# PJLab-ADG/nr3d_lib

Hardware: AMD Instinct MI355X
Metric: Mpoints/s LoTD fwd+bwd (16-lvl hash) + Mrays/s march+composite, 1 & 8 GPU (higher is better)
Workload: dtype f32; 1 GPU; configs[1]: 16-level Hash LoTD (gen_ngp_cfg: T=2^19, F=2, 6 Dense + 10 Hash), 2^20 points/GPU, fwd(+dy/dx) + dL/dx + dL/dparam, fp32; points_per_gpu=1048576, n_params=12131648, parallelism=single GPU

## Files before the change

### include/nr3d_hip.h

```cpp
#ifndef NR3D_HIP_H
#define NR3D_HIP_H
#include <stdint.h>

#ifdef __cplusplus
extern "C" {
#endif

enum { NR3D_F32 = 0, NR3D_F16 = 1, NR3D_F64 = 2, NR3D_I32 = 3, NR3D_I64 = 4, NR3D_U8 = 5, NR3D_I16 = 6, NR3D_I8 = 7 };

#define NR3D_ABI_VERSION 24

const char *nr3d_last_error(void);
int nr3d_abi_version(void);

enum {
	NR3D_PROF_LOTD_FWD = 0,
	NR3D_PROF_LOTD_FWD_LDS = 1,
	NR3D_PROF_LOTD_CONTRACT_DX = 2,
	NR3D_PROF_LOTD_BIN = 3,
	NR3D_PROF_LOTD_ACCUM = 4,
	NR3D_PROF_MARCH = 5,
	NR3D_PROF_COMPOSITE_FWD = 6,
	NR3D_PROF_COMPOSITE_BWD = 7,
	NR3D_PROF_LOTD_DIRECT = 8,
	NR3D_PROF_COUNT = 9
// ... 11 lines not shown
	NR3D_OPT_FWD_SPLIT = 6,
	NR3D_OPT_FWD_LDS_STAGE = 7,
	NR3D_OPT_HVP_LEVELS = 8,
	NR3D_OPT_HVP_PAIRLANE = 9,
	NR3D_OPT_HVP_SPLIT = 10,
	NR3D_OPT_VM_SPLIT = 11,
	NR3D_OPT_CP_DIRECT = 12,
	NR3D_OPT_MARCH_GROUP = 13,
	NR3D_OPT_PACK_SCAN = 14,
	NR3D_OPT_SORT_WAVE = 15,
	NR3D_OPT_VM_DIRECT = 16,
	NR3D_OPT_DIRECT_FIXED = 17,
	NR3D_OPT_VM_SORTED = 18,
	NR3D_OPT_MLP_X3 = 19,
	NR3D_OPT_PAIR_FOLD = 20,
	NR3D_OPT_COUNT = 21
};
int nr3d_set_option(int id, int64_t value);
int64_t nr3d_get_option(int id);

#define NR3D_LOTD_MAX_LEVELS 32
#define NR3D_LOTD_MAX_DIMS 4
#define NR3D_LOTD_MAX_PSEUDO 256

enum {
	NR3D_LOD_Dense = 0, NR3D_LOD_VectorMatrix = 1, NR3D_LOD_VecZMatXoY = 2, NR3D_LOD_CP = 3,
	NR3D_LOD_CPfast = 4, NR3D_LOD_NPlaneMul = 5, NR3D_LOD_NPlaneSum = 6, NR3D_LOD_Hash = 7
};

typedef struct nr3d_lotd_level {
	uint32_t res[NR3D_LOTD_MAX_DIMS];
// ... 37 lines not shown
                     void *dL_dy_T ,
                     int32_t max_level, void *fold ,
                     void *stream);

uint64_t nr3d_lotd_dparam_workspace_bytes(const nr3d_lotd_meta_t *meta, uint32_t n_points, uint32_t n_batches);
void nr3d_lotd_set_dparam_chunk_log2(int log2_points);

int nr3d_lotd_dLdy_feature_major(uint32_t n_points, uint32_t n_encoded_dims, int grad_dtype, const void *dL_dy,
                                 int64_t g_sn, int64_t g_se, float *out, void *stream);

int nr3d_lotd_half_params_ok(const nr3d_lotd_meta_t *meta, int batched);
int nr3d_lotd_pair_path_ok(const nr3d_lotd_meta_t *meta);
int nr3d_lotd_pair_direct_levels(const nr3d_lotd_meta_t *meta, uint32_t n_points);
uint64_t nr3d_lotd_fwd_lds_levels(const nr3d_lotd_meta_t *meta, uint32_t n_points);
uint64_t nr3d_lotd_pair_fold_bytes(const nr3d_lotd_meta_t *meta, uint32_t n_points, int32_t max_level);

int nr3d_lotd_bwd_dparam(const nr3d_lotd_meta_t *meta, const void *meta_dev, uint32_t n_points,
                         int grad_dtype, const void *dL_dy, int64_t dldy_sn, int64_t dldy_se,
                         const void *dL_ddLdx, const void *x, int param_dtype, const void *params,
                         const int64_t *batch_inds, const int64_t *batch_offsets, uint32_t batch_data_size, uint32_t n_batches,
                         int32_t min_level, int32_t max_level, int out_dtype, int assign, void *dL_dparam,
                         void *workspace, uint64_t workspace_bytes, void *fold, void *stream);

int nr3d_lotd_bwd_bwd_ddLdy(const nr3d_lotd_meta_t *meta, uint32_t n_points, int x_dtype, int param_dtype,
                            const void *dL_ddLdx, const void *dy_dx, int64_t dydx_sn, int64_t dydx_se,
                            void *dL_ddLdy, int64_t out_sn, int64_t out_se, void *stream);
uint64_t nr3d_lotd_bwd_bwd_dx_workspace_bytes(const nr3d_lotd_meta_t *meta, uint32_t n_points);
int nr3d_lotd_bwd_bwd_dx(const nr3d_lotd_meta_t *meta, const void *meta_dev, uint32_t n_points,
                         int x_dtype, int param_dtype, const void *dL_ddLdx,
                         const void *dL_dy, int64_t dldy_sn, int64_t dldy_se, const void *x,
// ... 377 lines not shown
```

### nr3d_lib_amd/_abi.py

```python
ABI_VERSION = 24
SIGNATURES = {
    'nr3d_abi_version': ('int', []),
    'nr3d_alpha_to_vw_backward': ('int', ['uint32_t', 'uint64_t', 'ptr', 'ptr', 'ptr', 'ptr', 'float', 'float', 'ptr', 'ptr']),
    'nr3d_alpha_to_vw_forward': ('int', ['uint32_t', 'uint64_t', 'ptr', 'ptr', 'float', 'float', 'ptr', 'ptr', 'ptr', 'ptr']),
    'nr3d_arange_num_steps': ('int', ['uint32_t', 'int', 'ptr', 'ptr', 'ptr', 'double', 'ptr', 'ptr']),
    'nr3d_forest_identify': ('int', ['ptr', 'uint64_t', 'ptr', 'ptr', 'ptr']),
    'nr3d_forest_ray_marching_count': ('int', ['ptr', 'uint32_t', 'ptr', 'ptr', 'ptr', 'ptr', 'ptr', 'ptr', 'ptr', 'ptr', 'ptr', 'ptr', 'float', 'float', 'float', 'uint32_t', 'ptr', 'ptr', 'ptr', 'ptr']),
    'nr3d_forest_ray_marching_emit': ('int', ['ptr', 'uint32_t', 'ptr', 'ptr', 'ptr', 'ptr', 'ptr', 'ptr', 'ptr', 'ptr', 'ptr', 'ptr', 'float', 'float', 'float', 'ptr', 'ptr', 'ptr', 'ptr', 'ptr', 'ptr', 'ptr']),
    'nr3d_freq_encode_bwd': ('int', ['uint64_t', 'uint32_t', 'uint32_t', 'uint32_t', 'ptr', 'ptr', 'int64_t', 'ptr', 'ptr']),
    'nr3d_freq_encode_bwd_bwd': ('int', ['uint64_t', 'uint32_t', 'uint32_t', 'uint32_t', 'ptr', 'ptr', 'ptr', 'int64_t', 'ptr', 'ptr', 'ptr']),
    'nr3d_freq_encode_fwd': ('int', ['uint64_t', 'uint32_t', 'uint32_t', 'uint32_t', 'ptr', 'ptr', 'int64_t', 'ptr']),
    'nr3d_get_option': ('int64_t', ['int']),
    'nr3d_interleave_linstep': ('int', ['uint32_t', 'int', 'ptr', 'ptr', 'ptr', 'double', 'double', 'ptr', 'ptr', 'ptr']),
    'nr3d_last_error': ('str', []),
    'nr3d_lotd_bwd_bwd_ddLdy': ('int', ['ptr', 'uint32_t', 'int', 'int', 'ptr', 'ptr', 'int64_t', 'int64_t', 'ptr', 'int64_t', 'int64_t', 'ptr']),
    'nr3d_lotd_bwd_bwd_dx': ('int', ['ptr', 'ptr', 'uint32_t', 'int', 'int', 'ptr', 'ptr', 'int64_t', 'int64_t', 'ptr', 'ptr', 'ptr', 'ptr', 'uint32_t', 'int32_t', 'ptr', 'ptr', 'uint64_t', 'ptr']),
    'nr3d_lotd_bwd_bwd_dx_workspace_bytes': ('uint64_t', ['ptr', 'uint32_t']),
    'nr3d_lotd_bwd_dparam': ('int', ['ptr', 'ptr', 'uint32_t', 'int', 'ptr', 'int64_t', 'int64_t', 'ptr', 'ptr', 'int', 'ptr', 'ptr', 'ptr', 'uint32_t', 'uint32_t', 'int32_t', 'int32_t', 'int', 'int', 'ptr', 'ptr', 'uint64_t', 'ptr', 'ptr']),
    'nr3d_lotd_bwd_dx': ('int', ['ptr', 'uint32_t', 'int', 'int', 'ptr', 'int64_t', 'int64_t', 'ptr', 'int64_t', 'int64_t', 'ptr', 'ptr', 'int32_t', 'ptr', 'ptr']),
    'nr3d_lotd_dLdy_feature_major': ('int', ['uint32_t', 'uint32_t', 'int', 'ptr', 'int64_t', 'int64_t', 'ptr', 'ptr']),
    'nr3d_lotd_dparam_workspace_bytes': ('uint64_t', ['ptr', 'uint32_t', 'uint32_t']),
    'nr3d_lotd_forest_bwd_bwd_dx': ('int', ['ptr', 'ptr', 'ptr', 'uint32_t', 'ptr', 'ptr', 'ptr', 'ptr', 'int', 'ptr', 'ptr', 'uint32_t', 'int32_t', 'ptr', 'ptr']),
    'nr3d_lotd_forest_bwd_dparam': ('int', ['ptr', 'ptr', 'ptr', 'uint32_t', 'ptr', 'ptr', 'ptr', 'ptr', 'int', 'ptr', 'ptr', 'uint32_t', 'int32_t', 'ptr', 'ptr', 'uint64_t', 'ptr']),
    'nr3d_lotd_forest_dparam_workspace_bytes': ('uint64_t', ['ptr', 'uint32_t', 'uint32_t']),
    'nr3d_lotd_forest_fwd': ('int', ['ptr', 'ptr', 'ptr', 'uint32_t', 'ptr', 'ptr', 'int', 'ptr', 'ptr', 'uint32_t', 'int32_t', 'ptr', 'int64_t', 'int64_t', 'ptr', 'int64_t', 'int64_t', 'ptr']),
    'nr3d_lotd_fwd': ('int', ['ptr', 'ptr', 'uint32_t', 'int', 'int', 'ptr', 'ptr', 'ptr', 'ptr', 'uint32_t', 'int32_t', 'ptr', 'int64_t', 'int64_t', 'ptr', 'int64_t', 'int64_t', 'ptr']),
    'nr3d_lotd_fwd_lds_levels': ('uint64_t', ['ptr', 'uint32_t']),
    'nr3d_lotd_grid_index': ('int', ['ptr', 'ptr', 'uint32_t', 'int', 'ptr', 'ptr', 'ptr', 'uint32_t', 'int32_t', 'ptr', 'ptr']),
    'nr3d_lotd_half_params_ok': ('int', ['ptr', 'int']),
    'nr3d_lotd_meta_create': ('int', ['int32_t', 'uint32_t', 'ptr', 'ptr', 'ptr', 'uint32_t', 'int', 'ptr']),
    'nr3d_lotd_meta_regroup': ('int', ['ptr', 'uint32_t', 'uint32_t', 'ptr']),
    'nr3d_lotd_pair_direct_levels': ('int', ['ptr', 'uint32_t']),
    'nr3d_lotd_pair_fold_bytes': ('uint64_t', ['ptr', 'uint32_t', 'int32_t']),
    'nr3d_lotd_pair_path_ok': ('int', ['ptr']),
    'nr3d_lotd_set_dparam_chunk_log2': ('void', ['int']),
    'nr3d_march_composite_bwd': ('int', ['uint32_t', 'ptr', 'ptr', 'ptr', 'ptr', 'ptr', 'float', 'float', 'int', 'ptr', 'ptr', 'ptr', 'ptr', 'ptr', 'ptr', 'ptr', 'ptr', 'ptr', 'ptr', 'uint64_t', 'ptr', 'ptr']),
    'nr3d_march_composite_fwd': ('int', ['uint32_t', 'ptr', 'ptr', 'ptr', 'ptr', 'ptr', 'ptr', 'ptr', 'int', 'float', 'float', 'float', 'uint32_t', 'ptr', 'ptr', 'ptr', 'ptr', 'ptr', 'ptr', 'uint64_t', 'uint64_t', 'ptr', 'ptr', 'ptr', 'ptr', 'ptr', 'ptr', 'ptr', 'ptr', 'uint64_t', 'ptr', 'float', 'float', 'int', 'ptr', 'ptr', 'ptr', 'ptr', 'ptr', 'ptr']),
    'nr3d_march_finish_samples': ('int', ['uint64_t', 'ptr', 'ptr', 'ptr', 'ptr', 'ptr', 'ptr', 'ptr', 'ptr', 'ptr']),
    'nr3d_mark_pack_boundaries': ('int', ['uint64_t', 'int', 'ptr', 'ptr', 'ptr']),
    'nr3d_merge_pack_union': ('int', ['uint32_t', 'ptr', 'ptr', 'uint32_t', 'ptr', 'ptr', 'ptr', 'ptr', 'ptr', 'ptr', 'ptr', 'ptr', 'ptr', 'ptr', 'ptr', 'ptr']),
    'nr3d_mlp_backward': ('int', ['ptr', 'uint64_t', 'ptr', 'int64_t', 'int64_t', 'ptr', 'int64_t', 'ptr', 'ptr', 'int64_t', 'int64_t', 'ptr', 'ptr', 'ptr']),
    'nr3d_mlp_backward_backward': ('int', ['ptr', 'uint64_t', 'ptr', 'int64_t', 'int64_t', 'ptr', 'int64_t', 'ptr', 'int64_t', 'int64_t', 'ptr', 'ptr', 'int64_t', 'ptr', 'ptr']),
    'nr3d_mlp_backward_backward_ok': ('int', ['ptr']),
    'nr3d_mlp_backward_packed_floats': ('uint64_t', ['ptr']),
    'nr3d_mlp_forward': ('int', ['ptr', 'uint64_t', 'ptr', 'int64_t', 'int64_t', 'ptr', 'ptr', 'int64_t', 'ptr']),
    'nr3d_mlp_half_backward': ('int', ['ptr', 'uint64_t', 'ptr', 'int64_t', 'int64_t', 'ptr', 'int64_t', 'ptr', 'ptr', 'int64_t', 'int64_t', 'ptr', 'ptr', 'ptr']),
    'nr3d_mlp_half_backward_packed_bytes': ('uint64_t', ['ptr']),
    'nr3d_mlp_half_forward': ('int', ['ptr', 'uint64_t', 'ptr', 'int64_t', 'int64_t', 'ptr', 'ptr', 'int64_t', 'ptr']),
# ... 75 lines not shown
```

### nr3d_lib_amd/_hip.py

```python
import ctypes as C
import os
import subprocess
import threading

import torch

from nr3d_lib_amd import _abi

_PKG = os.path.dirname(os.path.abspath(__file__))
LIB_PATH = os.path.join(_PKG, "libnr3d_hip.so")
ABI_VERSION = _abi.ABI_VERSION
CSRC = os.path.join(_PKG, "csrc")

F32, F16, F64, I32, I64, U8, I16, I8 = range(8)
DTYPE_CODE = {
    torch.float32: F32, torch.float16: F16, torch.float64: F64, torch.int32: I32, torch.int64: I64,
    torch.uint8: U8, torch.bool: U8, torch.int16: I16, torch.int8: I8,
}

_lib = None
_lock = threading.Lock()


def build(verbose=False, jobs=None):
# ... 91 lines not shown
def prof_enable(*names):
    mask = 0
    for n in names:
        mask |= 1 << PROF_IDS[n]
    lib().nr3d_prof_enable(mask)


def prof_read(name, reset=True):
    ms, n = C.c_double(0.0), C.c_uint32(0)
    check(lib().nr3d_prof_read(PROF_IDS[name], C.byref(ms), C.byref(n), 1 if reset else 0))
    return float(ms.value), int(n.value)


OPTION_IDS = dict(lotd_pair=0, pair_quad=1, pair_second=2, pair_direct=3, pair_fixed=4, fwd_pairlane=5, fwd_split=6,
                  fwd_lds_stage=7, hvp_levels=8, hvp_pairlane=9, hvp_split=10, vm_split=11, cp_direct=12, march_group=13,
                  pack_scan=14, sort_wave=15, vm_direct=16, direct_fixed=17, vm_sorted=18, mlp_x3=19, pair_fold=20)


def set_option(name, value):
    l = lib()
    check(l.nr3d_set_option(OPTION_IDS[name], -1 if value is None else int(value)))


def get_option(name):
    l = lib()
    return int(l.nr3d_get_option(OPTION_IDS[name]))


class options:

    def __init__(self, **kw):
# ... 193 lines not shown
```

### nr3d_lib_amd/bindings/_lotd.py

```python
import ctypes as C
import enum

import torch

from .. import _hip as H

MAX_LEVELS, MAX_DIMS, MAX_PSEUDO = 32, 4, 256


class LoDType(enum.IntEnum):
    Dense = 0
    VectorMatrix = 1
    VecZMatXoY = 2
    CP = 3
    CPfast = 4
    NPlaneMul = 5
    NPlaneSum = 6
    Hash = 7


class InterpolationType(enum.IntEnum):
    Linear = 0
    Smoothstep = 1

# ... 340 lines not shown
            if need_param_grad and level_buckets is not None and on_bucket is not None:
                for k, (lo, hi) in enumerate(level_buckets):
                    on_bucket(k, dL_dparam[m.level_offsets[int(lo)]:m.level_offsets[min(int(hi), m.n_levels - 1) + 1]])
            return (_cast(dL_dx, input.dtype), _cast(dL_dparam, params.dtype))
        g32 = dL_dy.detach() if native else _f32c(dL_dy.detach())
        gcode = H.F16 if native else H.F32
        gsn, gse = _strides2(g32)
        st = H.stream_of(input)
        tag = ("dx" if need_input_grad else "") + ("dp" if need_param_grad else "")
        with _Prof(m, f"LoTD{D}-bwd-{tag}", N):
            gT = fold = None
            if need_input_grad and N > 0:
                j, jsn, jse = _jac_view(dy_dx.detach(), N, E, D)
                if (need_param_grad and not batched and USE_BINNED_DPARAM and gse == 1 and gsn == E
                        and g32.data_ptr() % 16 == 0):
                    gT = H.empty((E, N), dtype=torch.float32, device=dev)
                    if typed:
                        nfold = H.lib().nr3d_lotd_pair_fold_bytes(C.byref(m._cmeta()), N, max_level)
                        if nfold:
                            fold = H.empty(((nfold + 3) // 4,), dtype=torch.int32, device=dev)
                H.check(H.lib().nr3d_lotd_bwd_dx(
                    C.byref(m._cmeta()), N, H.F32, gcode, H.ptr(g32), gsn, gse, H.ptr(j), jsn, jse, H.ptr(dL_dx), H.ptr(gT),
                    max_level, H.ptr(fold), st))
            if need_param_grad and N > 0:
                x32, (p32, pcode) = _f32c(input.detach()), _ptab(params)
                nbat = _n_batches(m, p32, batch_offsets, batched)
                ws, wsb = _dparam_workspace(m, N, dev, nbat)
                if gT is not None:
                    g32, gsn, gse, gcode = gT, 1, N, H.F32
                ranges = [(0, max_level)]
                if level_buckets is not None:
                    if batched:
                        raise RuntimeError("bwd: level_buckets need non-batched params")
                    if params.dtype != torch.float32:
                        raise RuntimeError("bwd: level_buckets need float params (the slices handed out are the result)")
# ... 119 lines not shown
```

### nr3d_lib_amd/csrc/host_api.hip

```cpp
#include "common.h"
#include <string.h>
#include <limits>
#include <chrono>
#include <mutex>
#include <vector>

namespace nr3d {

static thread_local char g_err[512] = {0};

char *err_buf() { return g_err; }

int fail(const char *fmt, ...) {
	va_list ap;
	va_start(ap, fmt);
	vsnprintf(g_err, sizeof(g_err), fmt, ap);
	va_end(ap);
	return 1;
}

namespace prof {
uint32_t g_mask = 0;
struct Pair { hipEvent_t a, b; };
static std::mutex g_mu;
// ... 12 lines not shown
	g_open[id] = p; g_is_open[id] = true;
}
void end(int id, hipStream_t st) {
	std::lock_guard<std::mutex> lk(g_mu);
	if (id < 0 || id >= NR3D_PROF_COUNT || !g_is_open[id]) return;
	g_is_open[id] = false;
	if (hipEventRecord(g_open[id].b, st) == hipSuccess) g_done[id].push_back(g_open[id]);
}
}

namespace opt {
static const int64_t kDefault[NR3D_OPT_COUNT] = {
	 1,  1,  1,  1,  1,  1,
	 1,  1,  1,  1,  1,  1,
	 1,  0,  1,  1,  1,  1,
	 1,  1,  1,
};
std::atomic<int64_t> g_val[NR3D_OPT_COUNT];
static const bool g_val_init = [] {
	for (int i = 0; i < NR3D_OPT_COUNT; ++i) g_val[i].store(kDefault[i], std::memory_order_relaxed);
	return true;
}();
}

}

using namespace nr3d;

extern "C" void nr3d_prof_enable(uint32_t mask) { prof::g_mask = mask; }

extern "C" int nr3d_prof_read(int id, double *total_ms, uint32_t *n_intervals, int reset) {
// ... 167 lines not shown
```

### nr3d_lib_amd/csrc/lotd.hip

```cpp
#include "lotd_device.h"
#include <stdlib.h>
#include <vector>
#include <type_traits>
#include <algorithm>

namespace nr3d {
namespace lotd {

template <typename YT> __device__ __forceinline__ void store_nt(YT *p, float v);

template <int D, int G, bool DYDX, bool DH, int ONLY = -1, typename PT = float>
__global__ __launch_bounds__(kBlock) void k_fwd(Sched s, const nr3d_lotd_meta_t *__restrict__ md, uint32_t N,
                                                int32_t max_level, uint32_t smooth, const float *__restrict__ x,
                                                const PT *__restrict__ params, Batch ba, uint32_t vec_ok,
                                                PT *__restrict__ y, int64_t y_sn, int64_t y_se,
                                                float *__restrict__ dydx, int64_t d_sn, int64_t d_se) {
	uint32_t q, chunk;
	if (!decode_block(s, blockIdx.x, q, chunk)) return;
	const uint32_t i = chunk * kBlock + threadIdx.x;
	if (i >= N) return;
	const uint32_t level = meta_level_of(md, q);
	const uint32_t foff0 = meta_cnt_of(md, q) * G;
	const uint32_t out0 = meta_col_of(md, q);

// ... 993 lines not shown
	for (uint32_t e = 0; e < E; ++e) {
		const float g = gy[(int64_t)e * g_se];
		const float *j = jj + (int64_t)e * d_se;
#pragma unroll
		for (int d = 0; d < D; ++d) acc[d] = __fmaf_rn(g, j[d], acc[d]);
	}
#pragma unroll
	for (int d = 0; d < D; ++d) dL_dx[(size_t)i * D + d] = acc[d];
}

template <int D, typename GT>
__global__ __launch_bounds__(kBlock) void k_contract_dx_rowmajor(uint32_t N, uint32_t E, const GT *__restrict__ dL_dy,
                                                                 const float *__restrict__ dydx, int64_t d_sn,
                                                                 int64_t d_se, float *__restrict__ dL_dx,
                                                                 float *__restrict__ dL_dy_T, uint32_t *__restrict__ fold,
                                                                 uint32_t gcols, uint32_t n_zero, uint32_t slot_off) {
	constexpr int TE = 32;
	__shared__ float tile[TE][kBlock + 1];
	__shared__ uint32_t gred[kBlock / 64];
	const uint32_t i0 = blockIdx.x * kBlock, i = i0 + threadIdx.x;
	const uint32_t n_here = min((uint32_t)kBlock, N - i0);
	uint32_t gbits = 0;
	auto gm = [&](uint32_t e, float v) { if (e < gcols) gbits = max(gbits, __float_as_uint(v) & 0x7FFFFFFFu); };
	if (fold && blockIdx.x == 0)
		for (uint32_t k = threadIdx.x; k < n_zero; k += kBlock) fold[k] = 0u;
	float acc[D];
#pragma unroll
	for (int d = 0; d < D; ++d) acc[d] = 0.0f;
	for (uint32_t e0 = 0; e0 < E; e0 += TE) {
		const uint32_t te = min((uint32_t)TE, E - e0);
		if (te == TE && (E & 3u) == 0u) {
// ... 14 lines not shown
				}
			}
		} else {
			for (uint32_t v = threadIdx.x; v < kBlock * te; v += kBlock) {
				const uint32_t p = v / te, e = v - p * te;
				if (p < n_here) {
					tile[e][p] = to_f32<GT>(dL_dy[(size_t)(i0 + p) * E + e0 + e]);
					if (fold) gm(e0 + e, tile[e][p]);
				}
			}
		}
		__syncthreads();
		if (dL_dy_T && i < N) {
#pragma unroll 8
			for (uint32_t e = 0; e < te; ++e) __builtin_nontemporal_store(tile[e][threadIdx.x], &dL_dy_T[(size_t)(e0 + e) * N + i]);
		}
		if (i < N) {
			const float *jj = dydx + (int64_t)i * d_sn + (int64_t)e0 * d_se;
#pragma unroll 8
			for (uint32_t e = 0; e < te; ++e) {
				const float g = tile[e][threadIdx.x];
				const float *j = jj + (int64_t)e * d_se;
#pragma unroll
				for (int d = 0; d < D; ++d) acc[d] = __fmaf_rn(g, __builtin_nontemporal_load(j + d), acc[d]);
			}
		}
		__syncthreads();
	}
	if (i < N) {
#pragma unroll
// ... 381 lines not shown
}

extern "C" int nr3d_lotd_bwd_dx(const nr3d_lotd_meta_t *meta, uint32_t N, int x_dtype, int param_dtype, const void *dL_dy,
                                int64_t g_sn, int64_t g_se, const void *dy_dx, int64_t d_sn, int64_t d_se, void *dL_dx,
                                void *dL_dy_T, int32_t max_level, void *fold_buf, void *stream) {
	NR3D_CHECK(meta != nullptr, "LoTD: meta is NULL");
	NR3D_CHECK(x_dtype == NR3D_F32 && (param_dtype == NR3D_F32 || param_dtype == NR3D_F16), "LoTD::bwd_dx: f32 x, f32 / f16 dL_dy");
	if (N == 0) return 0;
	NR3D_CHECK(dL_dy && dy_dx && dL_dx, "LoTDEncoding::bwd: need `dy_dx` to comput `dL_dx`.");
	const uint32_t E = meta->n_encoded_dims;
	const bool g_half = param_dtype == NR3D_F16;
	const bool row_major = (g_se == 1 && g_sn == (int64_t)E && ((uintptr_t)dL_dy % (g_half ? 8 : 16)) == 0);
	NR3D_CHECK(dL_dy_T == nullptr || row_major, "LoTD::bwd_dx: dL_dy_T needs a contiguous, 16-byte aligned [N, E] dL_dy");
	NR3D_CHECK(!g_half || (row_major && (E & 3u) == 0u), "LoTD::bwd_dx: half dL_dy must be a contiguous [N, E] tensor, E % 4 == 0");
	uint32_t gcols = 0, n_zero = 0, slot_off = 0;
	uint32_t *fold = (fold_buf && pair_fold_layout(meta, N, max_level, gcols, n_zero, slot_off) != 0) ? (uint32_t *)fold_buf : nullptr;
	NR3D_CHECK(!fold || row_major, "LoTD::bwd_dx: the hand-over buffer needs a contiguous, 16-byte aligned [N, E] dL_dy");
	prof::Scope ps(NR3D_PROF_LOTD_CONTRACT_DX, (hipStream_t)stream);
	DISPATCH_D(meta->n_dims_to_encode, {
		if (row_major && g_half)
			hipLaunchKernelGGL((k_contract_dx_rowmajor<D, __half>), dim3(div_up(N, kBlock)), dim3(kBlock), 0, (hipStream_t)stream, N, E,
			                   (const __half *)dL_dy, (const float *)dy_dx, d_sn, d_se, (float *)dL_dx, (float *)dL_dy_T, fold, gcols,
			                   n_zero, slot_off);
		else if (row_major)
			hipLaunchKernelGGL((k_contract_dx_rowmajor<D, float>), dim3(div_up(N, kBlock)), dim3(kBlock), 0, (hipStream_t)stream, N, E,
			                   (const float *)dL_dy, (const float *)dy_dx, d_sn, d_se, (float *)dL_dx, (float *)dL_dy_T, fold, gcols,
			                   n_zero, slot_off);
		else
			hipLaunchKernelGGL(k_contract_dx<D>, dim3(div_up(N, kBlock)), dim3(kBlock), 0, (hipStream_t)stream, N, E,
			                   (const float *)dL_dy, g_sn, g_se, (const float *)dy_dx, d_sn, d_se, (float *)dL_dx);
	});
	NR3D_LAUNCH_CHECK();
	return 0;
}

extern "C" uint64_t nr3d_lotd_pair_fold_bytes(const nr3d_lotd_meta_t *meta, uint32_t N, int32_t max_level) {
	uint32_t gcols, n_zero, slot_off;
	return meta ? pair_fold_layout(meta, N, max_level, gcols, n_zero, slot_off) : 0;
}

extern "C" int nr3d_lotd_bwd_dparam(const nr3d_lotd_meta_t *meta, const void *meta_dev, uint32_t N, int grad_dtype,
                                    const void *dL_dy, int64_t g_sn, int64_t g_se, const void *dL_ddLdx, const void *x,
// ... 216 lines not shown
```

### nr3d_lib_amd/csrc/lotd_bin.hip

```cpp
#include "lotd_vm.h"
#include "lotd_sorted.h"
#include <stdlib.h>
#include <type_traits>

#ifndef NR3D_BIN_LDS_KB
#define NR3D_BIN_LDS_KB 72
#define NR3D_BIN_MAX_BP 512
#endif
namespace nr3d {
namespace lotd {

constexpr int kAccThreads = 1024;
constexpr int kLdsDoubles = 16384;
constexpr int kRedSlots = 4;
#ifndef NR3D_BALLOT_RANK_BUCKETS
#define NR3D_BALLOT_RANK_BUCKETS 4
#endif
constexpr uint32_t kBallotRankBuckets = NR3D_BALLOT_RANK_BUCKETS;
constexpr int kMaxPlanLevels = 64;
constexpr uint32_t kMaxBuckets = 8192;
constexpr int kBinLdsDyn = NR3D_BIN_LDS_KB * 1024 + (int)(kMaxBuckets + 1) * 4;

#define DISPATCH_DG_BIN(D_, G_, ...)                                                 \
	do {                                                                             \
// ... 1519 lines not shown
		                    : p.dL_dy + (int64_t)p0 * p.g_sn;
		c.gc = c.g_rows;
		c.sn = p.g_sn; c.se = p.g_se;
		c.ba = p.batch;
		if (c.ba.inds) c.ba.inds += p0;
		c.ba.first_point = p0;
		bool gt_ready = !row_major;
		auto need_gt = [&]() {
			if (gt_ready) return;
			if (p.g_half) launch_transpose<__half>(n, E, reinterpret_cast<const __half *>(c.g_rows), p.g_sn, p.g_se, c.gt, p.st);
			else launch_transpose<float>(n, E, c.g_rows, p.g_sn, p.g_se, c.gt, p.st);
			c.gc = c.gt; c.sn = 1; c.se = (int64_t)n;
			gt_ready = true;
		};
		if (use_pair) {
			need_gt();
			NR3D_TRY(pair_chunk(p, c));
			continue;
		}
		uint64_t served = 0;
		if (plain) {
			CpPlan cp;
			uint32_t max_acc = 0;
			if ((served = cp_plan(meta, n, p.min_level, p.max_level, lay.part_bytes / 4, cp, max_acc))) {
				need_gt();
				NR3D_TRY(cp_direct_route(p, c, cp, max_acc));
			}
		}
		if (!p.g_half) {
			VsPlan vsp;
			const uint64_t smask = vm_sorted_plan(meta, n, p.n_batches, forest, p.min_level, p.max_level, served, vsp);
// ... 33 lines not shown
```

### nr3d_lib_amd/csrc/lotd_device.h

```cpp
#pragma once
#include "common.h"
#include <type_traits>

namespace nr3d {
namespace lotd {

constexpr int kBlock = 256;
constexpr uint32_t kPrimes[7] = {1u, 2654435761u, 805459861u, 3674653429u, 2097192037u, 1434869437u, 2165219737u};

constexpr int kSchedSegs = 16;
struct Sched {
	uint32_t n_chunks, n_pseudo, mode, n_slots;
	uint64_t skip;
	uint32_t seg_cum[8][kSchedSegs + 1];
	uint32_t seg_begin[8][kSchedSegs];
	uint32_t seg_q[8][kSchedSegs];
};

__device__ __forceinline__ bool decode_block_raw(const Sched &s, uint32_t b, uint32_t &q, uint32_t &chunk);
__device__ __forceinline__ bool decode_block(const Sched &s, uint32_t b, uint32_t &q, uint32_t &chunk) {
	if (!decode_block_raw(s, b, q, chunk)) return false;
	return s.mode == 3 || q >= 64u || !((s.skip >> q) & 1ull);
}
__device__ __forceinline__ bool decode_block_raw(const Sched &s, uint32_t b, uint32_t &q, uint32_t &chunk) {
// ... 657 lines not shown
	p.min_level = 0; p.max_level = 0x7fffffff;
	p.dparam = (float *)dparam; p.out_half = false; p.assign = false;
	p.workspace = nullptr; p.workspace_bytes = 0; p.st = nullptr;
	p.forest = nullptr; p.fold = nullptr;
	return p;
}

int dparam_binned(const DparamPass &pass, bool &handled);
bool dparam_one_pass(uint32_t n_points);

bool pair_applies(const nr3d_lotd_meta_t *m);
uint32_t pair_direct_levels(const nr3d_lotd_meta_t *m, uint32_t n_points);
void pair_layout(const nr3d_lotd_meta_t *m, uint32_t n_chunk, uint64_t &rec_bytes, uint64_t &offs_bytes, uint64_t &plan_bytes,
                 uint64_t &part_bytes);
int pair_chunk(const DparamPass &p, DparamChunk &c);
uint64_t pair_fold_layout(const nr3d_lotd_meta_t *m, uint32_t n, int32_t max_level, uint32_t &gcols, uint32_t &zero_words,
                          uint32_t &slot_off);

}
}
```

### nr3d_lib_amd/csrc/lotd_pair.hip

```cpp
#include "lotd_device.h"
#include <stdlib.h>


namespace nr3d {
namespace lotd {

constexpr uint32_t kPEpbMax = 8192;
constexpr int kPAccThreads = 1024;
constexpr int kPLdsMax = 2 * (int)kPEpbMax;
constexpr int kPMaxLv = 32;
constexpr uint32_t kPMaxNb = 511;
typedef uint32_t u32x4 __attribute__((ext_vector_type(4)));

struct PairPlan {
	uint32_t qmap[kPMaxLv];
	uint32_t nb[kPMaxLv];
	uint32_t epb[kPMaxLv];
	uint32_t shift[kPMaxLv];
	uint32_t bucket_base[kPMaxLv + 1];
	uint32_t offs_base[kPMaxLv];
	uint32_t n_blk, n_pseudo;
	uint32_t cap;
	uint32_t lg;
	uint32_t sum_log2;
// ... 274 lines not shown
	__syncthreads();
	if (threadIdx.x == 0) {
		uint32_t m = 0;
#pragma unroll
		for (int k = 0; k < kPBP / 64; ++k) m = max(m, scan_lds[k]);
		if (m > __hip_atomic_load(gmax, __ATOMIC_RELAXED, __HIP_MEMORY_SCOPE_AGENT)) atomicMax(gmax, m);
	}
}

template <int kPBP, bool SECOND = false>
__global__ __launch_bounds__(kPBP, kPBP == 768 ? 6 : 8)  void k_pair_bin(PairPlan plan, const nr3d_lotd_meta_t *__restrict__ md, uint32_t n,
                                                   int32_t max_level, uint32_t smooth, const float *__restrict__ x,
                                                   const float *__restrict__ g, int64_t g_sn, int64_t g_se,
                                                   u32x4 *__restrict__ rec, uint32_t *__restrict__ offs_g,
                                                   uint32_t *__restrict__ gmax, DirectPlan dp, const float *__restrict__ vin_,
                                                   uint32_t quad_on) {
	constexpr uint32_t kPCap = (uint32_t)kPBP * 4u;
	extern __shared__ __attribute__((aligned(16))) uint32_t smem[];
	__shared__ uint32_t scan_lds[kPBP / 64];
	u32x4 *stage = reinterpret_cast<u32x4 *>(smem);
	uint32_t *hist = smem + (size_t)kPCap * 4;
	const uint32_t blk = blockIdx.x, ql = blockIdx.y;
	const uint32_t q = plan.qmap[ql], nb = plan.nb[ql];
	const uint32_t level = meta_level_of(md, q);
	const Lvl L = load_level(md, level);
	const uint32_t i = blk * kPBP + threadIdx.x;
	for (uint32_t b = threadIdx.x; b <= nb; b += kPBP) hist[b] = 0;
	__syncthreads();
	const bool active = (i < n) && ((int32_t)level <= max_level);
	float xp[3] = {0.0f, 0.0f, 0.0f}, vin[3] = {0.0f, 0.0f, 0.0f}, g0 = 0.0f, g1 = 0.0f;
	if (active) {
#pragma unroll
		for (int d = 0; d < 3; ++d) xp[d] = x[(size_t)i * 3 + d];
		g0 = g[(int64_t)i * g_sn + (int64_t)(q * 2) * g_se];
		g1 = g[(int64_t)i * g_sn + (int64_t)(q * 2 + 1) * g_se];
		if constexpr (SECOND) {
#pragma unroll
// ... 361 lines not shown
#pragma unroll
		for (int k = 0; k < kFlush; ++k) if (p[k]) pair_st(p[k], old[k] + v[k], half_out);
	}
}

template <bool FIX, bool SECOND = false>
__global__ __launch_bounds__(kPAccThreads, 8) void k_pair_direct(DirectPlan dp, const nr3d_lotd_meta_t *__restrict__ md, uint32_t n,
                                                                 int32_t max_level, uint32_t smooth, const float *__restrict__ x,
                                                                 const float *__restrict__ g, int64_t g_sn, int64_t g_se,
                                                                 const uint32_t *__restrict__ gmax, float *__restrict__ partial,
                                                                 const float *__restrict__ vin_, uint32_t plan_rows, PairPlan plan,
                                                                 const uint32_t *__restrict__ offs_g, uint32_t n_units,
                                                                 uint32_t *__restrict__ tot, uint32_t *__restrict__ rep,
                                                                 uint32_t *__restrict__ item_start, uint32_t *__restrict__ ticket,
                                                                 const uint32_t *__restrict__ slots, uint32_t n_slots,
                                                                 uint32_t *__restrict__ gmax_out, uint32_t empty_one) {
	extern __shared__ __attribute__((aligned(16))) unsigned long long acc_raw[];
	__shared__ uint32_t queue[kPAccThreads / 64][128];
	if (blockIdx.y >= gridDim.y - plan_rows) {
		const uint32_t bid = (blockIdx.y - (gridDim.y - plan_rows)) * gridDim.x + blockIdx.x, nblk = (plan.bucket_base[plan.n_pseudo] + 15u) / 16u;
		if (bid < nblk) pair_plan_block(plan, offs_g, n_units, tot, rep, item_start, ticket, bid, nblk, slots, n_slots, gmax_out, empty_one != 0u);
		return;
	}
	double *acc = reinterpret_cast<double *>(acc_raw);
	const uint32_t r = blockIdx.x, fb = blockIdx.y;
	uint32_t e = 0;
	while (e + 1 < dp.n && dp.bucket_base[e + 1] <= fb) ++e;
	const uint32_t b = fb - dp.bucket_base[e], q = dp.qmap[e];
	const uint32_t level = meta_level_of(md, q);
	const Lvl L = load_level(md, level);
	const uint32_t kPEpb = 1u << dp.lg, kPLds = 2u << dp.lg;
	PairFix fx = {1.0, 1.0, false};
	if constexpr (FIX) fx = slots ? pair_fix_bits(gmax_slots(slots, n_slots, &queue[0][0]), dp.sum_log2) : pair_fix(gmax, dp.sum_log2);
	const bool fix = FIX && fx.on;
	for (uint32_t t = threadIdx.x; t < kPLds; t += kPAccThreads) acc_raw[t] = 0ull;
	__syncthreads();
	if ((int32_t)level <= max_level) {
		const uint32_t p_lo = r * dp.pts_per_rep;
		auto process = [&](uint32_t i) {
			float xp[3];
#pragma unroll
			for (int d = 0; d < 3; ++d) xp[d] = x[(size_t)i * 3 + d];
			const float g0 = g[(int64_t)i * g_sn + (int64_t)(q * 2) * g_se], g1 = g[(int64_t)i * g_sn + (int64_t)(q * 2 + 1) * g_se];
			uint32_t hdr[4], bkt[4], cell[3];
			constexpr int kW = SECOND ? 3 : 0;
			float A[4][2], wp[SECOND ? 4 : 1], vin[3] = {0.0f, 0.0f, 0.0f};
			bool valid;
			if constexpr (SECOND) {
#pragma unroll
				for (int d = 0; d < 3; ++d) vin[d] = vin_[(size_t)i * 3 + d];
			}
			uint32_t qmask;
			float wy_unused;
			pair_records<SECOND>(L, dp.shift[e], dp.epb[e], dp.lg, xp, g0, g1, smooth != 0, hdr, bkt, A, wp, cell, dp.nb[e], valid, vin, qmask, wy_unused, false);
			float lo[4][2], hi[4][2];
#pragma unroll
			for (int m = 0; m < 4; ++m)
#pragma unroll
// ... 251 lines not shown
                 uint64_t &part_bytes) {
	PairPlan plan;
	uint64_t ow;
	pair_plan(m, n_chunk, 0, 0x7fffffff, plan, ow);
	const uint32_t NB = plan.bucket_base[plan.n_pseudo];
	rec_bytes = (uint64_t)plan.n_pseudo * plan.n_blk * plan.cap * 16;
	offs_bytes = ((ow * 4 + 255) / 256) * 256;
	plan_bytes = (((uint64_t)NB * 3 + 4) * 4 + 255) / 256 * 256;
	part_bytes = (uint64_t)(kPairUnits + NB + kDirectMaxWg) * (2u << plan.lg) * 4;
}

void launch_plan_items(uint32_t NB, uint32_t n_blk, uint32_t units, const uint32_t *tot, uint32_t *rep, uint32_t *item_start,
                       hipStream_t st);

constexpr uint32_t kFoldHead = 64;
uint64_t pair_fold_layout(const nr3d_lotd_meta_t *m, uint32_t n, int32_t max_level, uint32_t &gcols, uint32_t &zero_words,
                          uint32_t &slot_off) {
	gcols = zero_words = slot_off = 0;
	if (!opt::on(NR3D_OPT_PAIR_FOLD) || !m || !pair_applies(m) || n == 0 || max_level < 0 || !dparam_one_pass(n)) return 0;
	if (2u * m->n_pseudo_levels != m->n_encoded_dims) return 0;
	uint32_t nq = 0;
	while (nq < m->n_pseudo_levels && (int32_t)m->map_levels[nq] <= max_level) ++nq;
	for (uint32_t q = nq; q < m->n_pseudo_levels; ++q)
		if ((int32_t)m->map_levels[q] <= max_level) return 0;
	if (nq == 0) return 0;
	PairPlan pl;
	uint64_t ow;
	pair_plan(m, n, 0, max_level, pl, ow);
	gcols = 2u * nq;
	zero_words = kFoldHead + pl.bucket_base[pl.n_pseudo];
	slot_off = (zero_words + 63u) & ~63u;
	return (uint64_t)(slot_off + div_up(n, (uint32_t)kBlock)) * 4u;
}

int pair_chunk(const DparamPass &p, DparamChunk &c) {
	const nr3d_lotd_meta_t *meta = p.meta, *md = p.meta_dev;
	const uint32_t n = c.n, units = kPairUnits;
	const uint32_t out_flags = (p.out_half ? 1u : 0u) | (p.assign ? 2u : 0u);
	const int32_t min_level = p.min_level, max_level = p.max_level;
	const float *x = c.xc, *g = c.gc, *vin = p.second ? c.vc : nullptr;
	const int64_t g_sn = c.sn, g_se = c.se;
	uint32_t *offs = c.offs, *plan_buf = c.plan_buf, *fold = p.fold;
	float *dparam = p.dparam, *partial = c.partial;
	hipStream_t st = p.st;
	uint32_t f_gcols = 0, f_zero = 0, f_slot = 0;
	if (fold && (vin || min_level > 0 || pair_fold_layout(meta, n, max_level, f_gcols, f_zero, f_slot) == 0)) fold = nullptr;
	const uint32_t *slots = fold ? fold + f_slot : nullptr;
	const uint32_t n_slots = div_up(n, (uint32_t)kBlock);
	PairPlan pl;
	uint64_t ow;
	pair_plan(meta, n, min_level, max_level, pl, ow);
	if (pl.n_pseudo == 0) return 0;
	DirectPlan dp;
	dp.n = 0;
	const uint32_t NB_full = pl.bucket_base[pl.n_pseudo];
	{
		const uint64_t skip = pair_direct_plan(pl, n, dp);
		if (skip) pair_plan(meta, n, min_level, max_level, pl, ow, skip);
	}
	uint32_t nb_max = 0;
	for (uint32_t q = 0; q < pl.n_pseudo; ++q) nb_max = nb_max > pl.nb[q] ? nb_max : pl.nb[q];
	const uint32_t NB = pl.bucket_base[pl.n_pseudo];
	uint32_t *tot = plan_buf, *rep = plan_buf + NB, *item_start = plan_buf + 2 * (size_t)NB;
	uint32_t *gmax = fold ? fold : plan_buf + 3 * (size_t)NB + 2;
	uint32_t *bticket = fold ? fold + kFoldHead : nullptr;
	const size_t bin_lds_max = (size_t)kPairBp * 4 * 16 + (size_t)(kPMaxNb + 2) * 8;
	static LdsOnce once_bin, once_acc;
	NR3D_TRY(NR3D_LDS_LIMIT(once_bin, c.dev, (int)bin_lds_max, k_pair_bin<kPairBp>, k_pair_bin<kPairBp, true>));
	NR3D_TRY(NR3D_LDS_LIMIT(once_acc, c.dev, kPLdsMax * 8, k_pair_direct<true>, k_pair_direct<false>, k_pair_direct<true, true>,
	                        k_pair_direct<false, true>, k_pair_accum<kPairUnroll, false>, k_pair_accum<kPairUnroll, true>));
	if (!fold) NR3D_HIP_CHECK(hipMemsetAsync(gmax, 0, 2 * sizeof(uint32_t), st));
	const size_t bin_lds = (size_t)kPairBp * 4 * 16 + (size_t)(nb_max + 1) * 4;
	const uint32_t quad_on = (!vin && pair_quad_enabled()) ? 1u : 0u;
#define NR3D_PAIR_BIN(BP) if (vin) NR3D_PAIR_BIN_(BP, true); else NR3D_PAIR_BIN_(BP, false)
#define NR3D_PAIR_BIN_(BP, SEC) hipLaunchKernelGGL((k_pair_bin<BP, SEC>), dim3(pl.n_blk, pl.n_pseudo), dim3(BP), bin_lds, st, pl, md, n, max_level, \
	meta->interpolation_type, x, g, g_sn, g_se, (u32x4 *)c.rec, offs, fold ? nullptr : gmax, dp, vin, quad_on)
	{
		prof::Scope ps(NR3D_PROF_LOTD_BIN, st);
		NR3D_PAIR_BIN(kPairBp);
	}
#undef NR3D_PAIR_BIN
#undef NR3D_PAIR_BIN_
	float *dpart = partial + (size_t)(units + NB_full) * (2u << pl.lg);
	const uint32_t nbk_direct = dp.n ? dp.bucket_base[dp.n] : 0u;
	const bool plan_in_direct = fold && dp.n && pl.n_pseudo;
	const uint32_t plan_rows = plan_in_direct ? div_up(div_up(NB, 16u), dp.R) : 0u;
	const uint32_t empty_one = (fold && (out_flags & 2u)) ? 1u : 0u;
	if (dp.n) {
		prof::Scope ps(NR3D_PROF_LOTD_DIRECT, st);
		auto direct = [&](auto kern) {
			hipLaunchKernelGGL(kern, dim3(dp.R, nbk_direct + plan_rows), dim3(kPAccThreads), (size_t)(16u << pl.lg), st, dp, md, n, max_level,
			                   meta->interpolation_type, x, g, g_sn, g_se, gmax, dpart, vin, plan_rows, pl, offs, units, tot, rep, item_start,
			                   gmax + 1, slots, n_slots, fold, empty_one);
		};
		if (vin) { if (pair_fixed()) direct(k_pair_direct<true, true>); else direct(k_pair_direct<false, true>); }
		else     { if (pair_fixed()) direct(k_pair_direct<true, false>); else direct(k_pair_direct<false, false>); }
	}
	if (pl.n_pseudo == 0) {
		if (dp.n)
			hipLaunchKernelGGL(k_pair_direct_reduce, dim3(nbk_direct, (2u << pl.lg) / kPAccThreads), dim3(kPAccThreads), 0, st, dp, md, dpart,
			                   dparam, out_flags);
		NR3D_LAUNCH_CHECK();
		return 0;
	}
	if (!plan_in_direct)
		hipLaunchKernelGGL(k_pair_plan, dim3(div_up(NB, 16)), dim3(1024), 0, st, pl, offs, units, tot, rep, item_start, gmax + 1, slots, n_slots,
		                   fold, empty_one);
	const uint32_t n_dred = fold ? nbk_direct * ((2u << pl.lg) / kPAccThreads) : 0u;
// ... 17 lines not shown
```

Before: 1164 Mpoints/s.

## Skip feature-major dL/dy transpose for pair path; read row-major gradients in place

Adds a pair_inplace option, on by default. When it applies, the bwd_dx contraction kernel stops writing the full feature-major dL_dy_T and writes only the columns needed by the direct levels into the fold buffer. The bin kernel then reads the row-major gradient directly, using a remapped 1-D grid that keeps groups of 8 blocks per pseudo-level adjacent so neighbouring blocks reuse the same cache lines. The goal is to cut the full transpose write and its later re-read, at the cost of strided row-major gradient reads in binning and a larger fold buffer.

```diff
diff --git a/include/nr3d_hip.h b/include/nr3d_hip.h
--- a/include/nr3d_hip.h
+++ b/include/nr3d_hip.h
@@ -8,7 +8,7 @@
 
 enum { NR3D_F32 = 0, NR3D_F16 = 1, NR3D_F64 = 2, NR3D_I32 = 3, NR3D_I64 = 4, NR3D_U8 = 5, NR3D_I16 = 6, NR3D_I8 = 7 };
 
-#define NR3D_ABI_VERSION 24
+#define NR3D_ABI_VERSION 25
 
 const char *nr3d_last_error(void);
 int nr3d_abi_version(void);
@@ -50,7 +50,8 @@
 	NR3D_OPT_VM_SORTED = 18,
 	NR3D_OPT_MLP_X3 = 19,
 	NR3D_OPT_PAIR_FOLD = 20,
-	NR3D_OPT_COUNT = 21
+	NR3D_OPT_PAIR_INPLACE = 21,
+	NR3D_OPT_COUNT = 22
 };
 int nr3d_set_option(int id, int64_t value);
 int64_t nr3d_get_option(int id);
@@ -118,6 +119,7 @@
 int nr3d_lotd_pair_direct_levels(const nr3d_lotd_meta_t *meta, uint32_t n_points);
 uint64_t nr3d_lotd_fwd_lds_levels(const nr3d_lotd_meta_t *meta, uint32_t n_points);
 uint64_t nr3d_lotd_pair_fold_bytes(const nr3d_lotd_meta_t *meta, uint32_t n_points, int32_t max_level);
+uint64_t nr3d_lotd_pair_inplace_calls(void);
 
 int nr3d_lotd_bwd_dparam(const nr3d_lotd_meta_t *meta, const void *meta_dev, uint32_t n_points,
                          int grad_dtype, const void *dL_dy, int64_t dldy_sn, int64_t dldy_se,
diff --git a/nr3d_lib_amd/_abi.py b/nr3d_lib_amd/_abi.py
--- a/nr3d_lib_amd/_abi.py
+++ b/nr3d_lib_amd/_abi.py
@@ -1,4 +1,4 @@
-ABI_VERSION = 24
+ABI_VERSION = 25
 SIGNATURES = {
     'nr3d_abi_version': ('int', []),
     'nr3d_alpha_to_vw_backward': ('int', ['uint32_t', 'uint64_t', 'ptr', 'ptr', 'ptr', 'ptr', 'float', 'float', 'ptr', 'ptr']),
@@ -32,6 +32,7 @@
     'nr3d_lotd_meta_regroup': ('int', ['ptr', 'uint32_t', 'uint32_t', 'ptr']),
     'nr3d_lotd_pair_direct_levels': ('int', ['ptr', 'uint32_t']),
     'nr3d_lotd_pair_fold_bytes': ('uint64_t', ['ptr', 'uint32_t', 'int32_t']),
+    'nr3d_lotd_pair_inplace_calls': ('uint64_t', []),
     'nr3d_lotd_pair_path_ok': ('int', ['ptr']),
     'nr3d_lotd_set_dparam_chunk_log2': ('void', ['int']),
     'nr3d_march_composite_bwd': ('int', ['uint32_t', 'ptr', 'ptr', 'ptr', 'ptr', 'ptr', 'float', 'float', 'int', 'ptr', 'ptr', 'ptr', 'ptr', 'ptr', 'ptr', 'ptr', 'ptr', 'ptr', 'ptr', 'uint64_t', 'ptr', 'ptr']),
diff --git a/nr3d_lib_amd/_hip.py b/nr3d_lib_amd/_hip.py
--- a/nr3d_lib_amd/_hip.py
+++ b/nr3d_lib_amd/_hip.py
@@ -129,7 +129,7 @@
 
 OPTION_IDS = dict(lotd_pair=0, pair_quad=1, pair_second=2, pair_direct=3, pair_fixed=4, fwd_pairlane=5, fwd_split=6,
                   fwd_lds_stage=7, hvp_levels=8, hvp_pairlane=9, hvp_split=10, vm_split=11, cp_direct=12, march_group=13,
-                  pack_scan=14, sort_wave=15, vm_direct=16, direct_fixed=17, vm_sorted=18, mlp_x3=19, pair_fold=20)
+                  pack_scan=14, sort_wave=15, vm_direct=16, direct_fixed=17, vm_sorted=18, mlp_x3=19, pair_fold=20, pair_inplace=21)
 
 
 def set_option(name, value):
diff --git a/nr3d_lib_amd/bindings/_lotd.py b/nr3d_lib_amd/bindings/_lotd.py
--- a/nr3d_lib_amd/bindings/_lotd.py
+++ b/nr3d_lib_amd/bindings/_lotd.py
@@ -378,11 +378,12 @@
                 j, jsn, jse = _jac_view(dy_dx.detach(), N, E, D)
                 if (need_param_grad and not batched and USE_BINNED_DPARAM and gse == 1 and gsn == E
                         and g32.data_ptr() % 16 == 0):
-                    gT = H.empty((E, N), dtype=torch.float32, device=dev)
                     if typed:
                         nfold = H.lib().nr3d_lotd_pair_fold_bytes(C.byref(m._cmeta()), N, max_level)
                         if nfold:
                             fold = H.empty(((nfold + 3) // 4,), dtype=torch.int32, device=dev)
+                    if not (fold is not None and not native and H.get_option("pair_inplace")):
+                        gT = H.empty((E, N), dtype=torch.float32, device=dev)
                 H.check(H.lib().nr3d_lotd_bwd_dx(
                     C.byref(m._cmeta()), N, H.F32, gcode, H.ptr(g32), gsn, gse, H.ptr(j), jsn, jse, H.ptr(dL_dx), H.ptr(gT),
                     max_level, H.ptr(fold), st))
diff --git a/nr3d_lib_amd/csrc/host_api.hip b/nr3d_lib_amd/csrc/host_api.hip
--- a/nr3d_lib_amd/csrc/host_api.hip
+++ b/nr3d_lib_amd/csrc/host_api.hip
@@ -50,7 +50,7 @@
 	 1,  1,  1,  1,  1,  1,
 	 1,  1,  1,  1,  1,  1,
 	 1,  0,  1,  1,  1,  1,
-	 1,  1,  1,
+	 1,  1,  1,  1,
 };
 std::atomic<int64_t> g_val[NR3D_OPT_COUNT];
 static const bool g_val_init = [] {
diff --git a/nr3d_lib_amd/csrc/lotd.hip b/nr3d_lib_amd/csrc/lotd.hip
--- a/nr3d_lib_amd/csrc/lotd.hip
+++ b/nr3d_lib_amd/csrc/lotd.hip
@@ -1031,7 +1031,7 @@
                                                                  const float *__restrict__ dydx, int64_t d_sn,
                                                                  int64_t d_se, float *__restrict__ dL_dx,
                                                                  float *__restrict__ dL_dy_T, uint32_t *__restrict__ fold,
-                                                                 uint32_t gcols, uint32_t n_zero, uint32_t slot_off) {
+                                                                 uint32_t gcols, uint32_t n_zero, uint32_t slot_off, FoldCols cols) {
 	constexpr int TE = 32;
 	__shared__ float tile[TE][kBlock + 1];
 	__shared__ uint32_t gred[kBlock / 64];
@@ -1076,6 +1076,13 @@
 		if (dL_dy_T && i < N) {
 #pragma unroll 8
 			for (uint32_t e = 0; e < te; ++e) __builtin_nontemporal_store(tile[e][threadIdx.x], &dL_dy_T[(size_t)(e0 + e) * N + i]);
+		}
+		if (fold && i < N) {
+			float *hand = reinterpret_cast<float *>(fold + cols.off);
+			for (uint32_t k = 0; k < cols.n; ++k) {
+				const uint32_t e = cols.col[k] - e0;
+				if (e < te) hand[(size_t)k * N + i] = tile[e][threadIdx.x];
+			}
 		}
 		if (i < N) {
 			const float *jj = dydx + (int64_t)i * d_sn + (int64_t)e0 * d_se;
@@ -1487,18 +1494,20 @@
 	NR3D_CHECK(dL_dy_T == nullptr || row_major, "LoTD::bwd_dx: dL_dy_T needs a contiguous, 16-byte aligned [N, E] dL_dy");
 	NR3D_CHECK(!g_half || (row_major && (E & 3u) == 0u), "LoTD::bwd_dx: half dL_dy must be a contiguous [N, E] tensor, E % 4 == 0");
 	uint32_t gcols = 0, n_zero = 0, slot_off = 0;
-	uint32_t *fold = (fold_buf && pair_fold_layout(meta, N, max_level, gcols, n_zero, slot_off) != 0) ? (uint32_t *)fold_buf : nullptr;
+	FoldCols cols;
+	uint32_t *fold = (fold_buf && pair_fold_layout(meta, N, max_level, gcols, n_zero, slot_off, &cols) != 0) ? (uint32_t *)fold_buf : nullptr;
+	if (!fold || g_half) cols.n = 0;
 	NR3D_CHECK(!fold || row_major, "LoTD::bwd_dx: the hand-over buffer needs a contiguous, 16-byte aligned [N, E] dL_dy");
 	prof::Scope ps(NR3D_PROF_LOTD_CONTRACT_DX, (hipStream_t)stream);
 	DISPATCH_D(meta->n_dims_to_encode, {
 		if (row_major && g_half)
 			hipLaunchKernelGGL((k_contract_dx_rowmajor<D, __half>), dim3(div_up(N, kBlock)), dim3(kBlock), 0, (hipStream_t)stream, N, E,
 			                   (const __half *)dL_dy, (const float *)dy_dx, d_sn, d_se, (float *)dL_dx, (float *)dL_dy_T, fold, gcols,
-			                   n_zero, slot_off);
+			                   n_zero, slot_off, cols);
 		else if (row_major)
 			hipLaunchKernelGGL((k_contract_dx_rowmajor<D, float>), dim3(div_up(N, kBlock)), dim3(kBlock), 0, (hipStream_t)stream, N, E,
 			                   (const float *)dL_dy, (const float *)dy_dx, d_sn, d_se, (float *)dL_dx, (float *)dL_dy_T, fold, gcols,
-			                   n_zero, slot_off);
+			                   n_zero, slot_off, cols);
 		else
 			hipLaunchKernelGGL(k_contract_dx<D>, dim3(div_up(N, kBlock)), dim3(kBlock), 0, (hipStream_t)stream, N, E,
 			                   (const float *)dL_dy, g_sn, g_se, (const float *)dy_dx, d_sn, d_se, (float *)dL_dx);
diff --git a/nr3d_lib_amd/csrc/lotd_bin.hip b/nr3d_lib_amd/csrc/lotd_bin.hip
--- a/nr3d_lib_amd/csrc/lotd_bin.hip
+++ b/nr3d_lib_amd/csrc/lotd_bin.hip
@@ -1557,7 +1557,7 @@
 			gt_ready = true;
 		};
 		if (use_pair) {
-			need_gt();
+			if (!pair_inplace_ok(p, c)) need_gt();
 			NR3D_TRY(pair_chunk(p, c));
 			continue;
 		}
diff --git a/nr3d_lib_amd/csrc/lotd_device.h b/nr3d_lib_amd/csrc/lotd_device.h
--- a/nr3d_lib_amd/csrc/lotd_device.h
+++ b/nr3d_lib_amd/csrc/lotd_device.h
@@ -695,8 +695,10 @@
 void pair_layout(const nr3d_lotd_meta_t *m, uint32_t n_chunk, uint64_t &rec_bytes, uint64_t &offs_bytes, uint64_t &plan_bytes,
                  uint64_t &part_bytes);
 int pair_chunk(const DparamPass &p, DparamChunk &c);
+bool pair_inplace_ok(const DparamPass &p, const DparamChunk &c);
+struct FoldCols { uint32_t n, off, col[16]; };
 uint64_t pair_fold_layout(const nr3d_lotd_meta_t *m, uint32_t n, int32_t max_level, uint32_t &gcols, uint32_t &zero_words,
-                          uint32_t &slot_off);
-
-}
-}
+                          uint32_t &slot_off, FoldCols *cols = nullptr);
+
+}
+}
diff --git a/nr3d_lib_amd/csrc/lotd_pair.hip b/nr3d_lib_amd/csrc/lotd_pair.hip
--- a/nr3d_lib_amd/csrc/lotd_pair.hip
+++ b/nr3d_lib_amd/csrc/lotd_pair.hip
@@ -1,5 +1,6 @@
 #include "lotd_device.h"
 #include <stdlib.h>
+#include <atomic>
 
 
 namespace nr3d {
@@ -312,13 +313,18 @@
                                                    const float *__restrict__ g, int64_t g_sn, int64_t g_se,
                                                    u32x4 *__restrict__ rec, uint32_t *__restrict__ offs_g,
                                                    uint32_t *__restrict__ gmax, DirectPlan dp, const float *__restrict__ vin_,
-                                                   uint32_t quad_on) {
+                                                   uint32_t quad_on, uint32_t rows_in_place) {
 	constexpr uint32_t kPCap = (uint32_t)kPBP * 4u;
 	extern __shared__ __attribute__((aligned(16))) uint32_t smem[];
 	__shared__ uint32_t scan_lds[kPBP / 64];
 	u32x4 *stage = reinterpret_cast<u32x4 *>(smem);
 	uint32_t *hist = smem + (size_t)kPCap * 4;
-	const uint32_t blk = blockIdx.x, ql = blockIdx.y;
+	uint32_t blk = blockIdx.x, ql = blockIdx.y;
+	if (rows_in_place) {
+		blk = (blockIdx.x / (8u * plan.n_pseudo)) * 8u + (blockIdx.x & 7u);
+		ql = (blockIdx.x >> 3) % plan.n_pseudo;
+		if (blk >= plan.n_blk) return;
+	}
 	const uint32_t q = plan.qmap[ql], nb = plan.nb[ql];
 	const uint32_t level = meta_level_of(md, q);
 	const Lvl L = load_level(md, level);
@@ -710,7 +716,8 @@
                                                                  uint32_t *__restrict__ tot, uint32_t *__restrict__ rep,
                                                                  uint32_t *__restrict__ item_start, uint32_t *__restrict__ ticket,
                                                                  const uint32_t *__restrict__ slots, uint32_t n_slots,
-                                                                 uint32_t *__restrict__ gmax_out, uint32_t empty_one) {
+                                                                 uint32_t *__restrict__ gmax_out, uint32_t empty_one,
+                                                                 uint32_t g_by_level) {
 	extern __shared__ __attribute__((aligned(16))) unsigned long long acc_raw[];
 	__shared__ uint32_t queue[kPAccThreads / 64][128];
 	if (blockIdx.y >= gridDim.y - plan_rows) {
@@ -737,7 +744,8 @@
 			float xp[3];
 #pragma unroll
 			for (int d = 0; d < 3; ++d) xp[d] = x[(size_t)i * 3 + d];
-			const float g0 = g[(int64_t)i * g_sn + (int64_t)(q * 2) * g_se], g1 = g[(int64_t)i * g_sn + (int64_t)(q * 2 + 1) * g_se];
+			const uint32_t gq = g_by_level ? e : q;
+			const float g0 = g[(int64_t)i * g_sn + (int64_t)(gq * 2) * g_se], g1 = g[(int64_t)i * g_sn + (int64_t)(gq * 2 + 1) * g_se];
 			uint32_t hdr[4], bkt[4], cell[3];
 			constexpr int kW = SECOND ? 3 : 0;
 			float A[4][2], wp[SECOND ? 4 : 1], vin[3] = {0.0f, 0.0f, 0.0f};
@@ -1019,9 +1027,11 @@
                        hipStream_t st);
 
 constexpr uint32_t kFoldHead = 64;
+static bool pair_inplace_enabled() { return opt::on(NR3D_OPT_PAIR_INPLACE); }
 uint64_t pair_fold_layout(const nr3d_lotd_meta_t *m, uint32_t n, int32_t max_level, uint32_t &gcols, uint32_t &zero_words,
-                          uint32_t &slot_off) {
+                          uint32_t &slot_off, FoldCols *cols) {
 	gcols = zero_words = slot_off = 0;
+	if (cols) cols->n = cols->off = 0;
 	if (!opt::on(NR3D_OPT_PAIR_FOLD) || !m || !pair_applies(m) || n == 0 || max_level < 0 || !dparam_one_pass(n)) return 0;
 	if (2u * m->n_pseudo_levels != m->n_encoded_dims) return 0;
 	uint32_t nq = 0;
@@ -1035,8 +1045,34 @@
 	gcols = 2u * nq;
 	zero_words = kFoldHead + pl.bucket_base[pl.n_pseudo];
 	slot_off = (zero_words + 63u) & ~63u;
-	return (uint64_t)(slot_off + div_up(n, (uint32_t)kBlock)) * 4u;
-}
+	uint64_t words = slot_off + div_up(n, (uint32_t)kBlock);
+	if (pair_inplace_enabled()) {
+		DirectPlan dp;
+		pair_direct_plan(pl, n, dp);
+		static_assert(2u * kDirectMaxLv <= sizeof(FoldCols::col) / sizeof(uint32_t), "FoldCols holds two columns per direct level");
+		const uint64_t off = (words + 3u) & ~(uint64_t)3u;
+		if (dp.n) {
+			if (cols) {
+				cols->n = 2u * dp.n; cols->off = (uint32_t)off;
+				for (uint32_t e = 0; e < dp.n; ++e) { cols->col[2 * e] = 2u * dp.qmap[e]; cols->col[2 * e + 1] = 2u * dp.qmap[e] + 1u; }
+			}
+			words = off + 2ull * dp.n * n;
+		}
+	}
+	return words * 4u;
+}
+
+static std::atomic<uint64_t> g_inplace_calls{0};
+static bool pair_inplace_input(const DparamPass &p, const DparamChunk &c) {
+	if (!p.fold || !pair_inplace_enabled() || p.second || p.g_half || p.min_level > 0 || c.n != p.N) return false;
+	const uint32_t E = p.meta->n_encoded_dims;
+	return c.gc == p.dL_dy && c.se == 1 && c.sn == (int64_t)E && E >= 2u && ((uintptr_t)c.gc & 15u) == 0;
+}
+bool pair_inplace_ok(const DparamPass &p, const DparamChunk &c) {
+	uint32_t gcols, zero, slot;
+	return pair_inplace_input(p, c) && pair_fold_layout(p.meta, c.n, p.max_level, gcols, zero, slot) != 0;
+}
+extern "C" uint64_t nr3d_lotd_pair_inplace_calls(void) { return g_inplace_calls.load(std::memory_order_relaxed); }
 
 int pair_chunk(const DparamPass &p, DparamChunk &c) {
 	const nr3d_lotd_meta_t *meta = p.meta, *md = p.meta_dev;
@@ -1049,7 +1085,10 @@
 	float *dparam = p.dparam, *partial = c.partial;
 	hipStream_t st = p.st;
 	uint32_t f_gcols = 0, f_zero = 0, f_slot = 0;
-	if (fold && (vin || min_level > 0 || pair_fold_layout(meta, n, max_level, f_gcols, f_zero, f_slot) == 0)) fold = nullptr;
+	FoldCols f_cols;
+	if (fold && (vin || min_level > 0 || pair_fold_layout(meta, n, max_level, f_gcols, f_zero, f_slot, &f_cols) == 0)) fold = nullptr;
+	const bool in_place = fold && pair_inplace_input(p, c);
+	if (in_place) g_inplace_calls.fetch_add(1, std::memory_order_relaxed);
 	const uint32_t *slots = fold ? fold + f_slot : nullptr;
 	const uint32_t n_slots = div_up(n, (uint32_t)kBlock);
 	PairPlan pl;
@@ -1078,8 +1117,9 @@
 	const size_t bin_lds = (size_t)kPairBp * 4 * 16 + (size_t)(nb_max + 1) * 4;
 	const uint32_t quad_on = (!vin && pair_quad_enabled()) ? 1u : 0u;
 #define NR3D_PAIR_BIN(BP) if (vin) NR3D_PAIR_BIN_(BP, true); else NR3D_PAIR_BIN_(BP, false)
-#define NR3D_PAIR_BIN_(BP, SEC) hipLaunchKernelGGL((k_pair_bin<BP, SEC>), dim3(pl.n_blk, pl.n_pseudo), dim3(BP), bin_lds, st, pl, md, n, max_level, \
-	meta->interpolation_type, x, g, g_sn, g_se, (u32x4 *)c.rec, offs, fold ? nullptr : gmax, dp, vin, quad_on)
+#define NR3D_PAIR_BIN_(BP, SEC) hipLaunchKernelGGL((k_pair_bin<BP, SEC>), bin_grid, dim3(BP), bin_lds, st, pl, md, n, max_level, \
+	meta->interpolation_type, x, g, g_sn, g_se, (u32x4 *)c.rec, offs, fold ? nullptr : gmax, dp, vin, quad_on, in_place ? 1u : 0u)
+	const dim3 bin_grid = in_place ? dim3(8u * div_up(pl.n_blk, 8u) * pl.n_pseudo) : dim3(pl.n_blk, pl.n_pseudo);
 	{
 		prof::Scope ps(NR3D_PROF_LOTD_BIN, st);
 		NR3D_PAIR_BIN(kPairBp);
@@ -1093,10 +1133,12 @@
 	const uint32_t empty_one = (fold && (out_flags & 2u)) ? 1u : 0u;
 	if (dp.n) {
 		prof::Scope ps(NR3D_PROF_LOTD_DIRECT, st);
+		const float *gd = in_place ? reinterpret_cast<const float *>(fold + f_cols.off) : g;
+		const int64_t gd_sn = in_place ? 1 : g_sn, gd_se = in_place ? (int64_t)n : g_se;
 		auto direct = [&](auto kern) {
 			hipLaunchKernelGGL(kern, dim3(dp.R, nbk_direct + plan_rows), dim3(kPAccThreads), (size_t)(16u << pl.lg), st, dp, md, n, max_level,
-			                   meta->interpolation_type, x, g, g_sn, g_se, gmax, dpart, vin, plan_rows, pl, offs, units, tot, rep, item_start,
-			                   gmax + 1, slots, n_slots, fold, empty_one);
+			                   meta->interpolation_type, x, gd, gd_sn, gd_se, gmax, dpart, vin, plan_rows, pl, offs, units, tot, rep, item_start,
+			                   gmax + 1, slots, n_slots, fold, empty_one, in_place ? 1u : 0u);
 		};
 		if (vin) { if (pair_fixed()) direct(k_pair_direct<true, true>); else direct(k_pair_direct<false, true>); }
 		else     { if (pair_fixed()) direct(k_pair_direct<true, false>); else direct(k_pair_direct<false, false>); }
```

New measurement: 1178 Mpoints/s, median of 4. 1.01x the previous value.
